# ZhaozhiQIAN/Hybrid-ODE-NeurIPS-2021

Measured on AMD Instinct MI355X. Metric: patient-trajectories/sec (fwd+adjoint) at dim=12, T=100, higher is better.
Workload: dtype f32; 1 GPU; dim12 synthetic, 10000 patients/GPU, T=100, dt=0.125, rk4(3/8), fused rhs+step kernel + discrete-adjoint kernel (split expert/learned wave pipelines); patients_total=10000, launch=hipGraph, lanes_per_patient=auto, theta_grad=True, parallelism=dp1, n_ranks=1, stage_tape=True

## Files before the change

hybrid-ode-neurips-2021_amd/csrc/hode_rk_split.hip:

```cpp
#include <hip/hip_runtime.h>
#include <stdlib.h>

#include "../../include/hode.h"
#include "hode_common.hpp"
#include "hode_host.hpp"
#include "hode_roche.hpp"

namespace hode {

#ifndef HODE_SPLIT_EXPERT_FIRST
#define HODE_SPLIT_EXPERT_FIRST 1
#endif
constexpr int kSplitPatients = 48;

struct SplitArgs {
  const float* __restrict__ t;
  const float* __restrict__ y0;
  const float* __restrict__ dosage;
  const float* __restrict__ dose_times;
  const float* __restrict__ theta;
  const float* __restrict__ w1;
  const float* __restrict__ b1;
  float* __restrict__ h;
  float* __restrict__ tape;
  unsigned long long* dbg;
  float* __restrict__ ltape;
  int* __restrict__ status;
  int B, T, K, perturb;
};

struct SpTimes {
  float t0, t1, dt, ts[4];
  HODE_DEV SpTimes(const float* __restrict__ t, int n, int perturb, int method) {
    t0 = t[n];
    t1 = t[n + 1];
    dt = t1 - t0;
    ts[0] = perturb ? nextafter_up(t0) : t0;
    ts[3] = perturb ? nextafter_down(t1) : t1;
    if (method == HODE_METHOD_RK4_38) {
      ts[1] = add_rn(t0, mul_rn(dt, (float)(1.0 / 3.0)));
      ts[2] = add_rn(t0, mul_rn(dt, (float)(2.0 / 3.0)));
    } else {
      ts[1] = add_rn(t0, mul_rn(0.5f, dt));
      ts[2] = ts[1];
    }
  }
};

template <int METHOD>
HODE_DEV float sp_stage_time(float t0, float t1, int perturb, int q) {
  const float dt = t1 - t0;
  const float c = METHOD == HODE_METHOD_RK4_38 ? (q == 1 ? (float)(1.0 / 3.0) : (q == 2 ? (float)(2.0 / 3.0) : 0.f))
                                               : (q == 0 ? 0.f : 0.5f);
  float tq = add_rn(t0, mul_rn(dt, c));
  tq = q == 3 ? t1 : tq;
  if (perturb) {
    if (q == 0) tq = nextafter_up(t0);
    if (q == 3) tq = nextafter_down(t1);
  }
  return tq;
}

constexpr int kSplitMaxT = 8192;
HODE_DEV void sp_stage_grid(float* __restrict__ tg, const float* __restrict__ t, int T) {
  for (int i = threadIdx.x; i < T + 3; i += blockDim.x) tg[i] = t[min(i, T - 1)];
}

template <int METHOD>
constexpr int sp_stages() { return METHOD == HODE_METHOD_EULER ? 1 : (METHOD == HODE_METHOD_MIDPOINT ? 2 : 4); }

template <int METHOD, class V>
HODE_DEV V sp_stage_state(int i, V y, float dt, V k1, V k2, V k3) {
  constexpr float c13 = (float)(1.0 / 3.0);
  if constexpr (METHOD == HODE_METHOD_MIDPOINT) return i == 0 ? y : vfma(k1, vsplat<V>(0.5f * dt), y);
  else if constexpr (METHOD == HODE_METHOD_RK4_38) {
    if (i == 0) return y;
    if (i == 1) return vfma(dt * k1, vsplat<V>(c13), y);
    if (i == 2) return vfma(vsplat<V>(dt), vfma(-k1, vsplat<V>(c13), k2), y);
    return vfma(vsplat<V>(dt), (k1 - k2) + k3, y);
  } else return y;
}
template <int METHOD, class V>
HODE_DEV V sp_advance(V y, float dt, V k1, V k2, V k3, V k4) {
  if constexpr (METHOD == HODE_METHOD_EULER) return vfma(vsplat<V>(dt), k1, y);
  else if constexpr (METHOD == HODE_METHOD_MIDPOINT) return vfma(vsplat<V>(dt), k2, y);
  else return vfma((k1 + 3.0f * (k2 + k3)) + k4, vsplat<V>(dt * 0.125f), y);
}

template <int V> struct IC { static constexpr int value = V; };

template <int MR> struct OwnSel { typedef float type; };
template <> struct OwnSel<2> { typedef f2 type; };

template <bool C, class A, class B> struct TypeSel { typedef A type; };
template <class A, class B> struct TypeSel<false, A, B> { typedef B type; };

#ifndef HODE_LTAPE_STAGES
#define HODE_LTAPE_STAGES 2
#endif
constexpr int kLearnedTapeStages = HODE_LTAPE_STAGES;
template <int METHOD> constexpr int sp_ltape_stages() { return METHOD == HODE_METHOD_RK4_38 ? kLearnedTapeStages : 0; }

template <int D>
struct MlRows {
  static constexpr int M = D - 4, MR = M / 4, DP = D / 2, MP = M / 2;
  static constexpr int NW = MR == 2 ? D : DP;
  static constexpr int NU = MR == 2 ? M : MP;
  static constexpr float kTanhScale = 2.885390081777927f;
  typedef typename OwnSel<MR>::type Own;
  typedef typename TypeSel<MR == 2, float, f2>::type Elem;
  struct Stage { Elem v[NW]; };
  struct Gath { Elem v[NU]; };
  f2 wp[NW];
  Own bias;
  HODE_DEV void load(const float* __restrict__ W, const float* __restrict__ b, int q) {
    if constexpr (MR == 2) {
#pragma unroll
      for (int i = 0; i < D; ++i) wp[i] = kTanhScale * pair2(W[(2 * q) * D + i], W[(2 * q + 1) * D + i]);
      bias = kTanhScale * pair2(b[2 * q], b[2 * q + 1]);
    } else {
#pragma unroll
      for (int ip = 0; ip < DP; ++ip) wp[ip] = kTanhScale * pair2(W[q * D + 2 * ip], W[q * D + 2 * ip + 1]);
      bias = kTanhScale * b[q];
    }
  }
  static HODE_DEV void gather(Own v, Elem* __restrict__ out) {
    if constexpr (MR == 2) {
      out[0] = quad_bcast<0>(v.x); out[1] = quad_bcast<0>(v.y);
      out[2] = quad_bcast<1>(v.x); out[3] = quad_bcast<1>(v.y);
      out[4] = quad_bcast<2>(v.x); out[5] = quad_bcast<2>(v.y);
      out[6] = quad_bcast<3>(v.x); out[7] = quad_bcast<3>(v.y);
    } else {
      out[0] = pair2(quad_bcast<0>(v), quad_bcast<1>(v));
      out[1] = pair2(quad_bcast<2>(v), quad_bcast<3>(v));
    }
  }
  static HODE_DEV Stage stage(const float4& e, Own Yo) {
    Stage Y;
    if constexpr (MR == 2) {
      Y.v[0] = e.x; Y.v[1] = e.y; Y.v[2] = e.z; Y.v[3] = e.w;
      gather(Yo, Y.v + 4);
    } else {
      Y.v[0] = pair2(e.x, e.y);
      Y.v[1] = pair2(e.z, e.w);
      gather(Yo, Y.v + 2);
    }
    return Y;
  }
  static HODE_DEV Own tanh_scaled(Own z) {
    if constexpr (MR == 2) {
      const f2 e = pair2(__builtin_amdgcn_exp2f(z.x), __builtin_amdgcn_exp2f(z.y)) + splat2(1.0f);
      return vfma(pair2(__builtin_amdgcn_rcpf(e.x), __builtin_amdgcn_rcpf(e.y)), splat2(-2.0f), splat2(1.0f));
    } else {
      return __builtin_fmaf(__builtin_amdgcn_rcpf(__builtin_amdgcn_exp2f(z) + 1.0f), -2.0f, 1.0f);
    }
  }
  HODE_DEV Own rhs(const Stage& Y) const {
    if constexpr (MR == 2) {
      f2 acc = bias, acc1 = splat2(0.f);
#pragma unroll
      for (int i = 0; i < D; i += 2) {
        acc = vfma(wp[i], Y.v[i], acc);
        acc1 = vfma(wp[i + 1], Y.v[i + 1], acc1);
      }
      return tanh_scaled(acc + acc1);
    } else {
      f2 acc = pair2(bias, 0.f);
#pragma unroll
      for (int ip = 0; ip < DP; ++ip) acc = vfma(wp[ip], Y.v[ip], acc);
      return tanh_scaled(hsum(acc));
    }
  }
  struct Part { f2 a, b; };
  HODE_DEV Part rhs_expert(const float4& e) const {
    Part p;
    if constexpr (MR == 2) {
      p.a = vfma(wp[2], e.z, vfma(wp[0], e.x, bias));
      p.b = vfma(wp[3], e.w, vfma(wp[1], e.y, splat2(0.f)));
    } else {
      p.a = vfma(wp[1], pair2(e.z, e.w), vfma(wp[0], pair2(e.x, e.y), pair2(bias, 0.f)));
      p.b = splat2(0.f);
    }
    return p;
  }
  HODE_DEV Own rhs_rest(const Part& p, const Stage& Y) const {
    if constexpr (MR == 2) {
      f2 acc = p.a, acc1 = p.b;
#pragma unroll
      for (int i = 4; i < D; i += 2) {
        acc = vfma(wp[i], Y.v[i], acc);
        acc1 = vfma(wp[i + 1], Y.v[i + 1], acc1);
      }
      return tanh_scaled(acc + acc1);
    } else {
      f2 acc = p.a;
#pragma unroll
      for (int ip = 2; ip < DP; ++ip) acc = vfma(wp[ip], Y.v[ip], acc);
      return tanh_scaled(hsum(acc));
    }
  }
  static HODE_DEV void outer_acc(f2 (&dw)[NW], Own u, const Stage& Y) {
#pragma unroll
    for (int i = 0; i < NW; ++i) dw[i] = vfma(u, Y.v[i], dw[i]);
  }
  static HODE_DEV float dw_at(const f2 (&dw)[NW], int r, int i) {
    if constexpr (MR == 2) return r == 0 ? dw[i].x : dw[i].y;
    else return (i & 1) ? dw[i / 2].y : dw[i / 2].x;
  }
  static HODE_DEV Own load_own(const float* __restrict__ src, int q) {
    if constexpr (MR == 2) {
      const float2 x = *reinterpret_cast<const float2*>(src + 4 + 2 * q);
      return pair2(x.x, x.y);
    } else return src[4 + q];
  }
  static HODE_DEV void store_own(float* __restrict__ dst, int q, Own v) {
    if constexpr (MR == 2) *reinterpret_cast<float2*>(dst + 4 + 2 * q) = make_float2(v.x, v.y);
    else dst[4 + q] = v;
  }
  template <int NL>
  static HODE_DEV void store_tape(float* __restrict__ dst, const Own* __restrict__ k) {
    if constexpr (MR == 2 && NL % 2 == 0) {
#pragma unroll
      for (int i = 0; i < NL; i += 2)
        *reinterpret_cast<float4*>(dst + 4 * (i / 2)) = make_float4(k[i].x, k[i].y, k[i + 1].x, k[i + 1].y);
    } else if constexpr (MR == 1 && NL == 4) {
      *reinterpret_cast<float4*>(dst) = make_float4(k[0], k[1], k[2], k[3]);
    } else if constexpr (MR == 1 && NL == 2) {
      *reinterpret_cast<float2*>(dst) = make_float2(k[0], k[1]);
    } else {
#pragma unroll
      for (int i = 0; i < NL; ++i) {
        if constexpr (MR == 2) *reinterpret_cast<float2*>(dst + 2 * i) = make_float2(k[i].x, k[i].y);
        else dst[i] = k[i];
      }
    }
  }
  template <int NL>
  static HODE_DEV void load_tape(const float* __restrict__ src, Own* __restrict__ k) {
    if constexpr (MR == 2 && NL % 2 == 0) {
#pragma unroll
      for (int i = 0; i < NL; i += 2) {
        const float4 v = *reinterpret_cast<const float4*>(src + 4 * (i / 2));
        k[i] = pair2(v.x, v.y); k[i + 1] = pair2(v.z, v.w);
      }
    } else if constexpr (MR == 1 && NL == 4) {
      const float4 v = *reinterpret_cast<const float4*>(src);
      k[0] = v.x; k[1] = v.y; k[2] = v.z; k[3] = v.w;
    } else if constexpr (MR == 1 && NL == 2) {
      const float2 v = *reinterpret_cast<const float2*>(src);
      k[0] = v.x; k[1] = v.y;
    } else {
#pragma unroll
      for (int i = 0; i < NL; ++i) {
        if constexpr (MR == 2) { const float2 v = *reinterpret_cast<const float2*>(src + 2 * i); k[i] = pair2(v.x, v.y); }
        else k[i] = src[i];
      }
    }
  }
};

template <int D, int METHOD, bool ABLATE, bool HILL2, bool K1, bool TAPE>
HODE_DEV void split_fwd_body(const SplitArgs& a) {
  constexpr int NS = sp_stages<METHOD>();
  typedef MlRows<D> Ml;
  typedef typename Ml::Own Own;
  constexpr int DP = Ml::DP;
  __shared__ __attribute__((aligned(16))) float ring[2][4][kSplitPatients][4];
  __shared__ __attribute__((aligned(16))) float dring[2][kSplitPatients][4];
  extern __shared__ float tg[];
  const int tid = threadIdx.x;
  const int wave = tid >> 6, lane = tid & 63;
  const int b0 = blockIdx.x * kSplitPatients;
  const RocheTheta th = load_theta(a.theta, ABLATE);
  const size_t row = (size_t)a.B * D;
  sp_stage_grid(tg, a.t, a.T);
#ifdef HODE_SPLIT_STAMPS
#define HODE_FSTAMP(k) if (a.dbg && blockIdx.x == 0 && lane == 0) a.dbg[(size_t)wave * a.T + (k)] = __builtin_amdgcn_s_memtime();
#else
#define HODE_FSTAMP(k)
#endif

  if (wave == 0) {
    const int slot = lane;
    const bool live = slot < kSplitPatients && b0 + slot < a.B;
    const int p = min(b0 + (slot < kSplitPatients ? slot : 0), a.B - 1);
    const int rslot = slot < kSplitPatients ? slot : 0;
    const unsigned lane_h = (unsigned)p * D, lane_t = (unsigned)p * 4;
    MlSlice<4, 1> none;
    float own1[1];
    f2 ya, yb;
    {
      const float4 v = *reinterpret_cast<const float4*>(a.y0 + (size_t)p * D);
      ya = pair2(v.x, v.y);
      yb = pair2(v.z, v.w);
      if (live) *reinterpret_cast<float4*>(a.h + (size_t)p * D) = v;
    }
    __syncthreads();
    auto e_iter = [&](int it, auto PAR) {
      constexpr int par = decltype(PAR)::value;
      if (it + 1 < a.T) {
        const float dt = tg[it + 1] - tg[it];
        const float4 dz = *reinterpret_cast<const float4*>(&dring[par][rslot][0]);
        const float dose[4] = {dz.x, dz.y, dz.z, dz.w};
        float* __restrict__ tape_it = TAPE ? a.tape + (size_t)it * (NS - 1) * a.B * 4 : nullptr;
        f2 ka[4], kb[4];
#pragma unroll
        for (int s = 0; s < 4; ++s) ka[s] = kb[s] = splat2(0.f);
#pragma unroll
        for (int s = 0; s < NS; ++s) {
          const f2 Ya = sp_stage_state<METHOD>(s, ya, dt, ka[0], ka[1], ka[2]);
          const f2 Yb = sp_stage_state<METHOD>(s, yb, dt, kb[0], kb[1], kb[2]);
          if (slot < kSplitPatients) *reinterpret_cast<float4*>(&ring[par][s][slot][0]) = make_float4(Ya.x, Ya.y, Yb.x, Yb.y);
          if constexpr (TAPE) {
            if (s >= 1)
              *reinterpret_cast<float4*>(tape_it + ((unsigned)(s - 1) * (unsigned)a.B * 4u + lane_t)) = make_float4(Ya.x, Ya.y, Yb.x, Yb.y);
          }
          const float Y[4] = {Ya.x, Ya.y, Yb.x, Yb.y};
          float k[4];
          roche_rhs<4, 1, ABLATE, HILL2>(th, none, dose[s], Y, k, own1);
          ka[s] = pair2(k[0], k[1]);
          kb[s] = pair2(k[2], k[3]);
        }
        ya = sp_advance<METHOD>(ya, dt, ka[0], ka[1], ka[2], ka[3]);
        yb = sp_advance<METHOD>(yb, dt, kb[0], kb[1], kb[2], kb[3]);
        *reinterpret_cast<float4*>(a.h + (size_t)(it + 1) * row + lane_h) = make_float4(ya.x, ya.y, yb.x, yb.y);
      }
      HODE_FSTAMP(it)
      __syncthreads();
    };
    for (int it = 0; it < a.T; it += 2) {
      e_iter(it, IC<0>{});
      if (it + 1 < a.T) e_iter(it + 1, IC<1>{});
    }
    if (a.status) {
      const bool bad = !(vfinite(ya) && vfinite(yb));
      if (bad && live) atomicOr(a.status, HODE_STATUS_NONFINITE);
    }
  } else {
    const int q = lane & 3;
    const int slot = (wave - 1) * 16 + (lane >> 2);
    const bool live = b0 + slot < a.B;
    const int p = min(b0 + slot, a.B - 1);
    Ml ml;
    ml.load(a.w1, a.b1, q);
    DoseSched<K1> ds;
    ds.dosage = a.dosage[p];
    ds.K = a.K;
    ds.taus = a.dose_times + (size_t)p * a.K;
    ds.tau0 = K1 ? ds.taus[0] : 0.f;
    auto dose_step = [&](int parity, float t0, float t1) {
      dring[parity][slot][q] = ds.at(sp_stage_time<METHOD>(t0, t1, a.perturb, q), th.kel).v;
    };
    if (a.T >= 2) dose_step(0, a.t[0], a.t[1]);
    if (a.T >= 3) dose_step(1, a.t[1], a.t[2]);
    Own yo = Ml::load_own(a.y0 + (size_t)p * D, q);
    if (live) Ml::store_own(a.h + (size_t)p * D, q, yo);
    constexpr int NLT = sp_ltape_stages<METHOD>();
    const size_t lt_step = (size_t)a.B * 4 * NLT * Ml::MR;
    const unsigned lt_lane = ((unsigned)p * 4 + q) * NLT * Ml::MR;
    __syncthreads();
    __syncthreads();
    auto m_iter = [&](int it, auto PAR) {
      constexpr int par = decltype(PAR)::value;
      const int n = it - 1;
      const float t_a = tg[it - 1], t_b = tg[it], t_c = tg[it + 1], t_d = tg[it + 2];
      const float dt = t_b - t_a;
      Own k[4];
      float4 e[4];
#pragma unroll
      for (int s = 0; s < NS; ++s) e[s] = *reinterpret_cast<const float4*>(&ring[par][s][slot][0]);
      __builtin_amdgcn_sched_barrier(0);
      dose_step(par, t_c, t_d);
#if HODE_SPLIT_EXPERT_FIRST
      typename Ml::Part pe[4];
#pragma unroll
      for (int s = 0; s < NS; ++s) pe[s] = ml.rhs_expert(e[s]);
#endif
#pragma unroll
      for (int s = 0; s < 4; ++s) k[s] = vsplat<Own>(0.f);
#pragma unroll
      for (int s = 0; s < NS; ++s) {
        const Own Yo = sp_stage_state<METHOD>(s, yo, dt, k[0], k[1], k[2]);
#if HODE_SPLIT_EXPERT_FIRST
        k[s] = ml.rhs_rest(pe[s], Ml::stage(e[s], Yo));
#else
        k[s] = ml.rhs(Ml::stage(e[s], Yo));
#endif
      }
      yo = sp_advance<METHOD>(yo, dt, k[0], k[1], k[2], k[3]);
      Ml::store_own(a.h + (size_t)(n + 1) * row + (size_t)p * D, q, yo);
      if constexpr (TAPE && NLT > 0) Ml::template store_tape<NLT>(a.ltape + (size_t)n * lt_step + lt_lane, k + (NS - NLT));
      HODE_FSTAMP(it)
      __syncthreads();
    };
    for (int it = 1; it < a.T; it += 2) {
      m_iter(it, IC<0>{});
      if (it + 1 < a.T) m_iter(it + 1, IC<1>{});
    }
    if (a.status) {
      if (!vfinite(yo) && live) atomicOr(a.status, HODE_STATUS_NONFINITE);
    }
  }
}

struct SplitBwdArgs {
  const float* __restrict__ t;
  const float* __restrict__ dosage;
  const float* __restrict__ dose_times;
  const float* __restrict__ theta;
  const float* __restrict__ w1;
  const float* __restrict__ b1;
  const float* __restrict__ h;
  const float* __restrict__ grad_h;
  float* __restrict__ grad_y0;
  float* __restrict__ part_ml;
  float* __restrict__ part_th;
  const float* __restrict__ tape;
  const float* __restrict__ ltape;
  int B, T, K, perturb;
  unsigned long long* dbg;
};

template <int METHOD, class V, class F>
HODE_DEV void sp_adjoint_step(V& lam, float dt, F&& vjp) {
  constexpr float c13 = (float)(1.0 / 3.0);
  if constexpr (METHOD == HODE_METHOD_EULER) {
    lam += vjp(0, dt * lam);
  } else if constexpr (METHOD == HODE_METHOD_MIDPOINT) {
    const V a1 = vjp(1, dt * lam);
    lam += a1;
    lam += vjp(0, (0.5f * dt) * a1);
  } else {
    const float w1 = dt * 0.125f, w3 = dt * 0.375f;
    const V a3 = vjp(3, w1 * lam);
    V da = dt * a3;
    V g1 = vfma(w1, lam, da);
    V g2 = vfma(w3, lam, -da);
    const V g = vfma(w3, lam, da);
    lam += a3;
    const V a2 = vjp(2, g);
    da = dt * a2;
    g2 += da;
    g1 = vfma(-c13, da, g1);
    lam += a2;
    const V a1 = vjp(1, g2);
    g1 = vfma(c13, dt * a1, g1);
    lam += a1;
    lam += vjp(0, g1);
  }
}

struct F4 {
  f2 a, b;
  HODE_DEV F4& operator+=(const F4& o) { a += o.a; b += o.b; return *this; }
  HODE_DEV F4 operator-() const { return F4{-a, -b}; }
};
HODE_DEV F4 operator*(float s, const F4& v) { return F4{s * v.a, s * v.b}; }
HODE_DEV F4 vfma(float s, const F4& x, const F4& y) { return F4{vfma(s, x.a, y.a), vfma(s, x.b, y.b)}; }

template <int D, bool CW>
struct SplitBwdShared {
  static constexpr int RD = CW ? 3 : 2;
  static constexpr int M = D - 4;
  float yring[RD][4][kSplitPatients][4];
  float cring[RD][4][kSplitPatients + 1][4];
  float dring[RD][kSplitPatients][8];
  float gring[RD][4][kSplitPatients + 1][4];
  float tdring[RD][kSplitPatients][8];
  float uring[CW ? RD : 1][4][CW ? kSplitPatients : 1][CW ? M : 1];
  float red[4][4][M * D + M];
};

template <int D, int METHOD, bool ABLATE, bool HILL2, bool NEED_TH, bool K1, bool TAPE>
HODE_DEV void split_bwd_body(const SplitBwdArgs& a, SplitBwdShared<D, TAPE>& sh) {
  constexpr int NS = sp_stages<METHOD>();
  typedef MlRows<D> Ml;
  typedef typename Ml::Own Own;
  constexpr int M = Ml::M, MR = Ml::MR, DP = Ml::DP, MP = Ml::MP;
  constexpr bool THW = TAPE && NEED_TH;
  constexpr bool CW = TAPE;
  constexpr int RD = SplitBwdShared<D, TAPE>::RD;
  constexpr int EL = CW ? 2 : 1;
  constexpr int CWAVE = THW ? 5 : 4;
  auto& yring = sh.yring; auto& cring = sh.cring; auto& dring = sh.dring; auto& gring = sh.gring;
  auto& tdring = sh.tdring; auto& uring = sh.uring; auto& red = sh.red;
  extern __shared__ float tg[];
  const int tid = threadIdx.x;
  const int wave = tid >> 6, lane = tid & 63;
  const int b0 = blockIdx.x * kSplitPatients;
  const RocheTheta th = load_theta(a.theta, ABLATE);
  const size_t row = (size_t)a.B * D;
  const int T = a.T;
  const int NIT = T + EL - 1;
  sp_stage_grid(tg, a.t, a.T);
#ifdef HODE_SPLIT_STAMPS
#define HODE_SSTAMP(k) if (a.dbg && blockIdx.x == 0 && lane == 0) a.dbg[(size_t)wave * (a.T + 2) + (k)] = __builtin_amdgcn_s_memtime();
#define HODE_PSTAMP(k, ph) { __builtin_amdgcn_sched_barrier(0); if (a.dbg && blockIdx.x == 0 && wave == 3 && lane == 0) a.dbg[(size_t)6 * (a.T + 2) + 64 + (size_t)(k) * 8 + (ph)] = __builtin_amdgcn_s_memtime(); __builtin_amdgcn_sched_barrier(0); }
  if (a.dbg && blockIdx.x < 8 && lane == 0) a.dbg[(size_t)6 * (a.T + 2) + blockIdx.x * 8 + wave] = __builtin_amdgcn_s_getreg(63492);
#else
#define HODE_SSTAMP(k)
#define HODE_PSTAMP(k, ph)
#endif
  auto run = [&](auto&& iter) {
    for (int k = 0; k < NIT; k += RD) {
      iter(k, IC<0>{});
      if (k + 1 < NIT) iter(k + 1, IC<1>{});
      if constexpr (RD == 3) {
        if (k + 2 < NIT) iter(k + 2, IC<2>{});
      }
    }
  };

  if (wave == 0) {
    const int slot = lane < kSplitPatients ? lane : 0;
    const bool mine = lane < kSplitPatients;
    const bool live = mine && b0 + slot < a.B;
    const int p = min(b0 + slot, a.B - 1);
    const float lv = live ? 1.0f : 0.0f;
    DoseSched<K1> ds;
    ds.dosage = a.dosage[p];
    ds.K = a.K;
    ds.taus = a.dose_times + (size_t)p * a.K;
    ds.tau0 = K1 ? ds.taus[0] : 0.f;
    const float ln_ec50 = log_f32(th.ec50);
    const int cslot = mine ? lane : kSplitPatients;
    if (lane < 16 * RD) (&cring[lane >> 4][(lane >> 2) & 3][kSplitPatients][0])[lane & 3] = 0.f;
    const unsigned lane_h = (unsigned)p * D, lane_t = (unsigned)p * 4;
    MlSlice<4, 1> none;
    MlColSlice<4, 1> nonec;
    GradAcc<4, 1> acc;
    acc.zero();
    float own1[1] = {0.f};

    float tp[4][4];
    auto fetch = [&](int m) {
      const float4 v = *reinterpret_cast<const float4*>(a.h + (size_t)m * row + lane_h);
      tp[0][0] = v.x; tp[0][1] = v.y; tp[0][2] = v.z; tp[0][3] = v.w;
      if constexpr (TAPE) {
        const float* __restrict__ tape_m = a.tape + (size_t)m * (NS - 1) * a.B * 4;
#pragma unroll
        for (int s = 1; s < NS; ++s) {
          const float4 u = *reinterpret_cast<const float4*>(tape_m + ((unsigned)(s - 1) * (unsigned)a.B * 4u + lane_t));
          tp[s][0] = u.x; tp[s][1] = u.y; tp[s][2] = u.z; tp[s][3] = u.w;
        }
      }
    };
    auto publish = [&](int m, int par) {
      if constexpr (TAPE) {
        if (mine) {
#pragma unroll
          for (int s = 0; s < NS; ++s)
            *reinterpret_cast<float4*>(&yring[par][s][slot][0]) = make_float4(tp[s][0], tp[s][1], tp[s][2], tp[s][3]);
        }
      } else {
        const SpTimes st(a.t, m, a.perturb, METHOD);
        const f2 ya = pair2(tp[0][0], tp[0][1]), yb = pair2(tp[0][2], tp[0][3]);
        f2 ka[4], kb[4];
#pragma unroll
        for (int s = 0; s < 4; ++s) ka[s] = kb[s] = splat2(0.f);
#pragma unroll
        for (int s = 0; s < NS; ++s) {
          const f2 Ya = sp_stage_state<METHOD>(s, ya, st.dt, ka[0], ka[1], ka[2]);
          const f2 Yb = sp_stage_state<METHOD>(s, yb, st.dt, kb[0], kb[1], kb[2]);
          const DoseVal dv = ds.at(st.ts[s], th.kel);
          if (mine) {
            *reinterpret_cast<float4*>(&yring[par][s][slot][0]) = make_float4(Ya.x, Ya.y, Yb.x, Yb.y);
            dring[par][slot][s] = dv.v;
            dring[par][slot][4 + s] = dv.dk;
          }
          if (s + 1 < NS) {
            const float Y[4] = {Ya.x, Ya.y, Yb.x, Yb.y};
            float k[4];
            roche_rhs<4, 1, ABLATE, HILL2>(th, none, dv.v, Y, k, own1);
            ka[s] = pair2(k[0], k[1]);
            kb[s] = pair2(k[2], k[3]);
          }
        }
      }
    };

    F4 lam;
    {
      const float4 g4 = *reinterpret_cast<const float4*>(a.grad_h + (size_t)(T - 1) * row + (size_t)p * D);
      lam.a = lv * pair2(g4.x, g4.y);
      lam.b = lv * pair2(g4.z, g4.w);
    }
    if (T >= 2) {
      fetch(T - 2);
      publish(T - 2, 0);
    }
    __syncthreads();
    auto e_iter = [&](int k, auto SI) {
      constexpr int S = decltype(SI)::value;
      constexpr int par = (S + 1) % RD;
      if (T - 3 - k >= 0) fetch(T - 3 - k);
      if (k >= EL && k <= T + EL - 2) {
        const int m = T - k + EL - 2;
        const float dt = tg[m + 1] - tg[m];
        float Y[4][4];
        F4 cs[4];
        DoseVal dv[4];
        {
          const float4 d0 = *reinterpret_cast<const float4*>(&dring[par][slot][0]);
          const float4 d1 = *reinterpret_cast<const float4*>(&dring[par][slot][4]);
          dv[0].v = d0.x; dv[1].v = d0.y; dv[2].v = d0.z; dv[3].v = d0.w;
          dv[0].dk = d1.x; dv[1].dk = d1.y; dv[2].dk = d1.z; dv[3].dk = d1.w;
          if constexpr (THW) {
            *reinterpret_cast<float4*>(&tdring[S][slot][0]) = d0;
            *reinterpret_cast<float4*>(&tdring[S][slot][4]) = d1;
          }
        }
#pragma unroll
        for (int s = 0; s < NS; ++s) {
          const float4 yv = *reinterpret_cast<const float4*>(&yring[par][s][slot][0]);
          const float4 cv = *reinterpret_cast<const float4*>(&cring[par][s][cslot][0]);
          Y[s][0] = yv.x; Y[s][1] = yv.y; Y[s][2] = yv.z; Y[s][3] = yv.w;
          cs[s].a = pair2(cv.x, cv.y);
          cs[s].b = pair2(cv.z, cv.w);
        }
        sp_adjoint_step<METHOD>(lam, dt, [&](int s, const F4& gs) {
          const float g[4] = {gs.a.x, gs.a.y, gs.b.x, gs.b.y};
          float av[4];
          if constexpr (THW) {
            if (mine) *reinterpret_cast<float4*>(&gring[S][s][slot][0]) = make_float4(g[0], g[1], g[2], g[3]);
          }
          roche_vjp<4, 1, ABLATE, HILL2, NEED_TH && !THW>(th, none, nonec, ln_ec50, dv[s], Y[s], own1, g, 0, av, acc);
          F4 r = cs[s];
          r.a += pair2(av[0], av[1]);
          r.b += pair2(av[2], av[3]);
          return r;
        });
        const float4 g4 = *reinterpret_cast<const float4*>(a.grad_h + (size_t)m * row + lane_h);
        lam.a = vfma(lv, pair2(g4.x, g4.y), lam.a);
        lam.b = vfma(lv, pair2(g4.z, g4.w), lam.b);
      }
      if (T - 3 - k >= 0) publish(T - 3 - k, par);
      HODE_SSTAMP(k)
      __syncthreads();
    };
    run(e_iter);
    if (live) *reinterpret_cast<float4*>(a.grad_y0 + (size_t)p * D) = make_float4(lam.a.x, lam.a.y, lam.b.x, lam.b.y);
    if constexpr (!THW) {
#pragma unroll
      for (int i = 0; i < kNTheta; ++i) {
        const float v = row_sum(NEED_TH ? acc.dth[i] : 0.f);
        if ((lane & 15) == 0) red[0][lane >> 4][i] = v;
      }
      __builtin_amdgcn_fence(__ATOMIC_SEQ_CST, "wavefront");
      if (lane < kNTheta)
        a.part_th[(size_t)blockIdx.x * kNTheta + lane] = (red[0][0][lane] + red[0][1][lane]) + (red[0][2][lane] + red[0][3][lane]);
    }
  } else if (THW && wave == 4) {
    const int slot = lane < kSplitPatients ? lane : 0;
    const bool mine = lane < kSplitPatients;
    const int p = min(b0 + slot, a.B - 1);
    const int gslot = mine ? lane : kSplitPatients;
    const float ln_ec50 = log_f32(th.ec50);
    if (lane < 16 * RD) (&gring[lane >> 4][(lane >> 2) & 3][kSplitPatients][0])[lane & 3] = 0.f;
    const unsigned lane_h = (unsigned)p * D, lane_t = (unsigned)p * 4;
    float dth[kNTheta];
#pragma unroll
    for (int i = 0; i < kNTheta; ++i) dth[i] = 0.f;
    float tp[4][4];
    auto fetch = [&](int m) {
      const float4 v = *reinterpret_cast<const float4*>(a.h + (size_t)m * row + lane_h);
      tp[0][0] = v.x; tp[0][1] = v.y; tp[0][2] = v.z; tp[0][3] = v.w;
      const float* __restrict__ tape_m = a.tape + (size_t)m * (NS - 1) * a.B * 4;
#pragma unroll
      for (int s = 1; s < NS; ++s) {
        const float4 u = *reinterpret_cast<const float4*>(tape_m + ((unsigned)(s - 1) * (unsigned)a.B * 4u + lane_t));
        tp[s][0] = u.x; tp[s][1] = u.y; tp[s][2] = u.z; tp[s][3] = u.w;
      }
    };
    auto theta_step = [&](int gpar) {
      const float4 d0 = *reinterpret_cast<const float4*>(&tdring[gpar][slot][0]);
      const float4 d1 = *reinterpret_cast<const float4*>(&tdring[gpar][slot][4]);
      const float dvv[4] = {d0.x, d0.y, d0.z, d0.w}, dvk[4] = {d1.x, d1.y, d1.z, d1.w};
#pragma unroll
      for (int si = 0; si < NS; ++si) {
        const int s = NS - 1 - si;
        const float4 gv = *reinterpret_cast<const float4*>(&gring[gpar][s][gslot][0]);
        DoseVal dv;
        dv.v = dvv[s]; dv.dk = dvk[s];
        const float g[4] = {gv.x, gv.y, gv.z, gv.w};
        roche_theta_grad<ABLATE, HILL2>(th, ln_ec50, dv, tp[s], g, dth);
      }
    };
    __syncthreads();
    auto t_iter = [&](int k, auto SI) {
      constexpr int S = decltype(SI)::value;
      constexpr int gpar = (S + RD - 1) % RD;
      if (k >= EL + 1) theta_step(gpar);
      if (k >= EL && T - k + EL - 2 >= 0) fetch(T - k + EL - 2);
      HODE_SSTAMP(k)
      __syncthreads();
    };
    run(t_iter);
    if (T >= 2) theta_step((NIT - 1) % RD);
#pragma unroll
    for (int i = 0; i < kNTheta; ++i) {
      const float v = row_sum(dth[i]);
      if ((lane & 15) == 0) red[0][lane >> 4][i] = v;
    }
    __builtin_amdgcn_fence(__ATOMIC_SEQ_CST, "wavefront");
    if (lane < kNTheta)
      a.part_th[(size_t)blockIdx.x * kNTheta + lane] = (red[0][0][lane] + red[0][1][lane]) + (red[0][2][lane] + red[0][3][lane]);
  } else if (CW && wave == CWAVE) {
    const int slot = lane < kSplitPatients ? lane : 0;
    const bool mine = lane < kSplitPatients;
    float wq[M][4];
#pragma unroll
    for (int j = 0; j < M; ++j)
#pragma unroll
      for (int q = 0; q < 4; ++q) wq[j][q] = a.w1[j * D + q];
    __syncthreads();
    auto c_iter = [&](int k, auto SI) {
      constexpr int S = decltype(SI)::value;
      constexpr int cpar = (S + RD - 1) % RD;
      if (k >= 1 && k - 1 <= T - 2) {
        float u[NS][M];
#pragma unroll
        for (int s = 0; s < NS; ++s) {
#pragma unroll
          for (int j4 = 0; j4 < M; j4 += 4) {
            const float4 v = *reinterpret_cast<const float4*>(&uring[cpar][s][slot][j4]);
            u[s][j4] = v.x; u[s][j4 + 1] = v.y; u[s][j4 + 2] = v.z; u[s][j4 + 3] = v.w;
          }
        }
        __builtin_amdgcn_sched_barrier(0);
#pragma unroll
        for (int s = 0; s < NS; ++s) {
          float c[4];
#pragma unroll
          for (int q = 0; q < 4; ++q) {
            if constexpr (MR == 2) {
              float cq = 0.f;
#pragma unroll
              for (int j = 0; j < M; ++j) cq = __builtin_fmaf(wq[j][q], u[s][j], cq);
              c[q] = cq;
            } else {
              float cx = 0.f, cy = 0.f;
#pragma unroll
              for (int jp = 0; jp < MP; ++jp) {
                cx = __builtin_fmaf(wq[2 * jp][q], u[s][2 * jp], cx);
                cy = __builtin_fmaf(wq[2 * jp + 1][q], u[s][2 * jp + 1], cy);
              }
              c[q] = cx + cy;
            }
          }
          if (mine) *reinterpret_cast<float4*>(&cring[cpar][s][slot][0]) = make_float4(c[0], c[1], c[2], c[3]);
        }
      }
      HODE_SSTAMP(k)
      __syncthreads();
    };
    run(c_iter);
  } else {
    const int q = lane & 3;
    const int slot = (wave - 1) * 16 + (lane >> 2);
    const bool live = b0 + slot < a.B;
    const int p = min(b0 + slot, a.B - 1);
    const float lv = live ? 1.0f : 0.0f;
    Ml ml;
    ml.load(a.w1, a.b1, q);
    typename Ml::Elem wc[Ml::NU];
    f2 wtp[Ml::NU];
    if constexpr (MR == 2) {
#pragma unroll
      for (int j = 0; j < M; ++j) {
        wc[j] = a.w1[j * D + q];
        wtp[j] = pair2(a.w1[j * D + 4 + 2 * q], a.w1[j * D + 4 + 2 * q + 1]);
      }
    } else {
#pragma unroll
      for (int jp = 0; jp < MP; ++jp) {
        wc[jp] = pair2(a.w1[(2 * jp) * D + q], a.w1[(2 * jp + 1) * D + q]);
        wtp[jp] = pair2(a.w1[(2 * jp) * D + 4 + q], a.w1[(2 * jp + 1) * D + 4 + q]);
      }
    }
    f2 dw[Ml::NW];
    Own db = vsplat<Own>(0.f);
#pragma unroll
    for (int i = 0; i < Ml::NW; ++i) dw[i] = splat2(0.f);
    DoseSched<K1> ds;
    ds.dosage = a.dosage[p];
    ds.K = a.K;
    ds.taus = a.dose_times + (size_t)p * a.K;
    ds.tau0 = K1 ? ds.taus[0] : 0.f;
    Own lam = lv * Ml::load_own(a.grad_h + (size_t)(T - 1) * row + (size_t)p * D, q);
    Own yo_nx, gh_nx;
    constexpr int NLT = TAPE ? sp_ltape_stages<METHOD>() : 0;
    const size_t lt_step = (size_t)a.B * 4 * NLT * MR;
    const unsigned lt_lane = ((unsigned)p * 4 + q) * NLT * MR;
    Own lt_nx[NLT > 0 ? NLT : 1], lt_n2[NLT > 0 ? NLT : 1];
    {
      const int m0 = T >= 2 ? T - 2 : 0;
      const int m1 = m0 >= 1 ? m0 - 1 : 0;
      yo_nx = Ml::load_own(a.h + (size_t)m0 * row + (size_t)p * D, q);
      gh_nx = Ml::load_own(a.grad_h + (size_t)m0 * row + (size_t)p * D, q);
      if constexpr (NLT > 0) {
        Ml::template load_tape<NLT>(a.ltape + (size_t)m0 * lt_step + lt_lane, lt_nx);
        Ml::template load_tape<NLT>(a.ltape + (size_t)m1 * lt_step + lt_lane, lt_n2);
      }
    }
    __syncthreads();
    auto m_iter = [&](int k, auto SI) {
      constexpr int par = decltype(SI)::value;
      if (k <= T - 2) {
        HODE_PSTAMP(k, 0)
        const int m = T - 2 - k;
        const float t0 = tg[m], t1 = tg[m + 1];
        const float dt = t1 - t0;
        const Own yo = yo_nx, gh = gh_nx;
        Own lt[NLT > 0 ? NLT : 1];
#pragma unroll
        for (int i = 0; i < NLT; ++i) { lt[i] = lt_nx[i]; lt_nx[i] = lt_n2[i]; }
        {
          const int mn = m >= 1 ? m - 1 : 0;
          yo_nx = Ml::load_own(a.h + (size_t)mn * row + (size_t)p * D, q);
          gh_nx = Ml::load_own(a.grad_h + (size_t)mn * row + (size_t)p * D, q);
          if constexpr (NLT > 0) Ml::template load_tape<NLT>(a.ltape + (size_t)(m >= 2 ? m - 2 : 0) * lt_step + lt_lane, lt_n2);
        }
        typename Ml::Stage Y[4];
        Own so[4];
        float4 e[4];
#pragma unroll
        for (int s = 0; s < NS; ++s) e[s] = *reinterpret_cast<const float4*>(&yring[par][s][slot][0]);
        __builtin_amdgcn_sched_barrier(0);
        HODE_PSTAMP(k, 1)
        if constexpr (TAPE) {
          const DoseVal dq = ds.at(sp_stage_time<METHOD>(t0, t1, a.perturb, q), th.kel);
          dring[par][slot][q] = dq.v;
          if constexpr (NEED_TH) dring[par][slot][4 + q] = dq.dk;
        }
#if HODE_SPLIT_EXPERT_FIRST
        typename Ml::Part pe[4];
#pragma unroll
        for (int s = 0; s < NS - NLT; ++s) pe[s] = ml.rhs_expert(e[s]);
#endif
#pragma unroll
        for (int s = 0; s < 4; ++s) so[s] = vsplat<Own>(0.f);
#pragma unroll
        for (int s = 0; s < NS; ++s) {
          const Own Yo = sp_stage_state<METHOD>(s, yo, dt, so[0], so[1], so[2]);
          Y[s] = Ml::stage(e[s], Yo);
          if (s >= NS - NLT) so[s] = lt[s - (NS - NLT) < 0 ? 0 : s - (NS - NLT)];
#if HODE_SPLIT_EXPERT_FIRST
          else so[s] = ml.rhs_rest(pe[s], Y[s]);
#else
          else so[s] = ml.rhs(Y[s]);
#endif
        }
        HODE_PSTAMP(k, 2)
        sp_adjoint_step<METHOD>(lam, dt, [&](int s, Own gs) {
          HODE_PSTAMP(k, 6 - s)
          const Own u = gs * vfma(-so[s], so[s], vsplat<Own>(1.0f));
          db += u;
          Ml::outer_acc(dw, u, Y[s]);
          if constexpr (CW) {
            if constexpr (MR == 2) *reinterpret_cast<float2*>(&uring[par][s][slot][2 * q]) = make_float2(u.x, u.y);
            else uring[par][s][slot][q] = u;
          }
          typename Ml::Gath uf;
          Ml::gather(u, uf.v);
          if constexpr (MR == 2) {
            float cq = 0.f;
            f2 av = splat2(0.f), av1 = splat2(0.f);
#pragma unroll
            for (int j = 0; j < M; j += 2) {
              if constexpr (!CW) cq = __builtin_fmaf(wc[j], uf.v[j], cq);
              av = vfma(wtp[j], uf.v[j], av);
              if constexpr (!CW) cq = __builtin_fmaf(wc[j + 1], uf.v[j + 1], cq);
              av1 = vfma(wtp[j + 1], uf.v[j + 1], av1);
            }
            if constexpr (!CW) cring[par][s][slot][q] = cq;
            return av + av1;
          } else {
            f2 c2 = splat2(0.f), a2 = splat2(0.f);
#pragma unroll
            for (int jp = 0; jp < MP; ++jp) {
              if constexpr (!CW) c2 = vfma(wc[jp], uf.v[jp], c2);
              a2 = vfma(wtp[jp], uf.v[jp], a2);
            }
            if constexpr (!CW) cring[par][s][slot][q] = hsum(c2);
            return hsum(a2);
          }
        });
        lam = vfma(lv, gh, lam);
        HODE_PSTAMP(k, 7)
      }
      HODE_SSTAMP(k)
      __syncthreads();
    };
    run(m_iter);
    if (live) Ml::store_own(a.grad_y0 + (size_t)p * D, q, lam);
    float* out = a.part_ml + ((size_t)blockIdx.x * 3 + (wave - 1)) * (M * D + M);
    const bool writer = (lane & 15) < 4;
    float* mine = &red[wave][lane >> 4][0];
#pragma unroll
    for (int r = 0; r < MR; ++r) {
#pragma unroll
      for (int i = 0; i < D; ++i) {
        const float v = row_sum_stride4(Ml::dw_at(dw, r, i));
        if (writer) mine[(q * MR + r) * D + i] = v;
      }
      float dbr;
      if constexpr (MR == 2) dbr = r == 0 ? db.x : db.y;
      else dbr = db;
      const float vb = row_sum_stride4(dbr);
      if (writer) mine[M * D + q * MR + r] = vb;
    }
    __builtin_amdgcn_fence(__ATOMIC_SEQ_CST, "wavefront");
    for (int c = lane; c < M * D + M; c += 64)
      out[c] = (red[wave][0][c] + red[wave][1][c]) + (red[wave][2][c] + red[wave][3][c]);
  }
}

__global__ __launch_bounds__(64) void split_fold_kernel(const float* __restrict__ part_ml, const float* __restrict__ part_th,
                                                        int nblk, int P_ml, int n_w, float* __restrict__ gw,
                                                        float* __restrict__ gb, float* __restrict__ gth, int need_th,
                                                        int overwrite) {
  const int j = blockIdx.x;
  const int lane = threadIdx.x;
  const bool ml = j < P_ml;
  const float* src = ml ? part_ml + j : part_th + (j - P_ml);
  const int rows = ml ? 3 * nblk : nblk;
  const int stride = ml ? P_ml : kNTheta;
  float s = 0.f;
  for (int base = 0; base < rows; base += 64 * 8) {
    float v[8];
#pragma unroll
    for (int q = 0; q < 8; ++q) {
      const int w = base + lane + 64 * q;
      v[q] = w < rows ? src[(size_t)w * stride] : 0.f;
    }
#pragma unroll
    for (int q = 0; q < 8; ++q) s += v[q];
  }
  s = wave_sum(s);
  if (lane != 0) return;
  float* dst = nullptr;
  if (ml) dst = j < n_w ? (gw ? gw + j : nullptr) : (gb ? gb + (j - n_w) : nullptr);
  else if (gth) dst = gth + (j - P_ml);
  if (!dst) return;
  if (!ml && !need_th) s = 0.f;
  *dst = overwrite ? s : *dst + s;
}

#ifndef HODE_SPLIT_WPE_FWD
#define HODE_SPLIT_WPE_FWD 2
#endif
#ifndef HODE_SPLIT_WPE_BWD
#define HODE_SPLIT_WPE_BWD 2
#endif
#ifndef HODE_SPLIT_WPE_BWD_MIN
#define HODE_SPLIT_WPE_BWD_MIN 1
#endif

template <int D, int METHOD, bool ABLATE, bool NEED_TH, bool TAPE>
__global__ __launch_bounds__(384) __attribute__((amdgpu_waves_per_eu(HODE_SPLIT_WPE_BWD_MIN, HODE_SPLIT_WPE_BWD))) void split_bwd_kernel(SplitBwdArgs a) {
  __shared__ __attribute__((aligned(16))) SplitBwdShared<D, TAPE> sh;
  const bool hill2 = ABLATE || (a.theta[0] == 2.0f && a.theta[1] == 2.0f);
  if (hill2 && a.K == 1) split_bwd_body<D, METHOD, ABLATE, true, NEED_TH, true, TAPE>(a, sh);
  else if (hill2) split_bwd_body<D, METHOD, ABLATE, true, NEED_TH, false, TAPE>(a, sh);
  else split_bwd_body<D, METHOD, ABLATE, false, NEED_TH, false, TAPE>(a, sh);
}

template <int D, int METHOD, bool ABLATE, bool TAPE>
__global__ __launch_bounds__(256) __attribute__((amdgpu_waves_per_eu(1, HODE_SPLIT_WPE_FWD))) void split_fwd_kernel(SplitArgs a) {
  const bool hill2 = ABLATE || (a.theta[0] == 2.0f && a.theta[1] == 2.0f);
  if (hill2 && a.K == 1) split_fwd_body<D, METHOD, ABLATE, true, true, TAPE>(a);
  else if (hill2) split_fwd_body<D, METHOD, ABLATE, true, false, TAPE>(a);
  else split_fwd_body<D, METHOD, ABLATE, false, false, TAPE>(a);
}

}

namespace {

template <int D, bool ABLATE>
int split_method(const hode_solve_desc* d, const hode::SplitArgs& a, hipStream_t s) {
  const dim3 grid((d->batch + hode::kSplitPatients - 1) / hode::kSplitPatients), block(256);
  const size_t lds = (size_t)(d->n_times + 3) * sizeof(float);
#define HODE_SPLIT_FWD(M)                                                                                 \
  if (a.tape) hipLaunchKernelGGL((hode::split_fwd_kernel<D, M, ABLATE, true>), grid, block, lds, s, a);   \
  else hipLaunchKernelGGL((hode::split_fwd_kernel<D, M, ABLATE, false>), grid, block, lds, s, a);
  switch (d->method) {
    case HODE_METHOD_EULER: HODE_SPLIT_FWD(HODE_METHOD_EULER) break;
    case HODE_METHOD_MIDPOINT: HODE_SPLIT_FWD(HODE_METHOD_MIDPOINT) break;
    default: HODE_SPLIT_FWD(HODE_METHOD_RK4_38) break;
  }
  return hode::hip_fail(hipGetLastError(), "split kernel launch");
}

}

namespace {

template <int D, bool ABLATE>
int split_bwd_method(const hode_solve_desc* d, const hode::SplitBwdArgs& a, hipStream_t s) {
  const dim3 grid((d->batch + hode::kSplitPatients - 1) / hode::kSplitPatients), block(256);
  const size_t lds = (size_t)(d->n_times + 3) * sizeof(float);
#define HODE_SPLIT_BWD(M)                                                                                        \
  if (d->need_theta_grad) {                                                                                      \
    if (a.tape) hipLaunchKernelGGL((hode::split_bwd_kernel<D, M, ABLATE, true, true>), grid, dim3(384), lds, s, a); \
    else hipLaunchKernelGGL((hode::split_bwd_kernel<D, M, ABLATE, true, false>), grid, block, lds, s, a);          \
  } else {                                                                                                       \
    if (a.tape) hipLaunchKernelGGL((hode::split_bwd_kernel<D, M, ABLATE, false, true>), grid, dim3(320), lds, s, a); \
    else hipLaunchKernelGGL((hode::split_bwd_kernel<D, M, ABLATE, false, false>), grid, block, lds, s, a);         \
  }
  switch (d->method) {
    case HODE_METHOD_EULER: HODE_SPLIT_BWD(HODE_METHOD_EULER) break;
    case HODE_METHOD_MIDPOINT: HODE_SPLIT_BWD(HODE_METHOD_MIDPOINT) break;
    default: HODE_SPLIT_BWD(HODE_METHOD_RK4_38) break;
  }
  return hode::hip_fail(hipGetLastError(), "split bwd kernel launch");
}

}

namespace hode {

bool split_supported(const hode_solve_desc* d) { return (d->latent_dim == 8 || d->latent_dim == 12) && d->n_times <= kSplitMaxT; }

static size_t al256s(size_t x) { return (x + 255) / 256 * 256; }

static int n_stages(int method) { return method == HODE_METHOD_EULER ? 1 : (method == HODE_METHOD_MIDPOINT ? 2 : 4); }

static size_t split_partials_bytes(const hode_solve_desc* d) {
  const size_t nblk = (d->batch + kSplitPatients - 1) / kSplitPatients;
  const size_t M = d->latent_dim - 4;
  return al256s(nblk * 3 * (M * d->latent_dim + M) * sizeof(float)) + al256s(nblk * kNTheta * sizeof(float));
}
static size_t split_etape_bytes(const hode_solve_desc* d) {
  if (!(d->flags & HODE_FLAG_TAPE) || d->n_times < 2) return 0;
  return al256s((size_t)(d->n_times - 1) * (n_stages(d->method) - 1) * d->batch * 4 * sizeof(float));
}
static size_t split_ltape_bytes(const hode_solve_desc* d) {
  if (!(d->flags & HODE_FLAG_TAPE) || d->n_times < 2 || n_stages(d->method) != 4 || kLearnedTapeStages == 0) return 0;
  return al256s((size_t)(d->n_times - 1) * d->batch * (d->latent_dim - 4) * kLearnedTapeStages * sizeof(float));
}
static size_t split_tape_bytes(const hode_solve_desc* d) { return split_etape_bytes(d) + split_ltape_bytes(d); }
size_t split_workspace_bytes(const hode_solve_desc* d) { return split_partials_bytes(d) + split_tape_bytes(d); }
static float* split_tape(const hode_solve_desc* d) {
  return split_etape_bytes(d) ? (float*)((char*)d->workspace + split_partials_bytes(d)) : nullptr;
}
static float* split_ltape(const hode_solve_desc* d) {
  return split_ltape_bytes(d) ? (float*)((char*)d->workspace + split_partials_bytes(d) + split_etape_bytes(d)) : nullptr;
}

int split_rk_bwd(const hode_solve_desc* d, hipStream_t s) {
  const int nblk = (d->batch + kSplitPatients - 1) / kSplitPatients;
  const int M = d->latent_dim - 4;
  const int Pml = M * d->latent_dim + M;
  char* ws = (char*)d->workspace;
  SplitBwdArgs a{};
  a.t = d->t; a.dosage = d->dosage; a.dose_times = d->dose_times; a.theta = d->theta; a.w1 = d->w1; a.b1 = d->b1;
  a.h = d->h; a.grad_h = d->grad_h; a.grad_y0 = d->grad_y0;
  a.part_ml = (float*)ws;
  a.part_th = (float*)(ws + al256s((size_t)nblk * 3 * Pml * sizeof(float)));
  a.B = d->batch; a.T = d->n_times; a.K = d->n_dose; a.perturb = d->perturb;
  a.tape = split_tape(d);
  a.ltape = split_ltape(d);
#ifdef HODE_SPLIT_STAMPS
  if (const char* env = getenv("HODE_SPLIT_DBG_PTR")) a.dbg = (unsigned long long*)strtoull(env, nullptr, 0);
#endif
  const bool abl = d->rhs_kind == HODE_RHS_ROCHE_ABLATE;
  int e;
  if (d->latent_dim == 8) e = abl ? split_bwd_method<8, true>(d, a, s) : split_bwd_method<8, false>(d, a, s);
  else e = abl ? split_bwd_method<12, true>(d, a, s) : split_bwd_method<12, false>(d, a, s);
  if (e || (d->flags & HODE_FLAG_SKIP_FOLD)) return e;
  const bool th_out = d->grad_theta != nullptr && (d->need_theta_grad || (d->flags & HODE_FLAG_OVERWRITE_GRADS));
  hipLaunchKernelGGL(split_fold_kernel, dim3(Pml + (th_out ? kNTheta : 0)), dim3(64), 0, s, a.part_ml, a.part_th, nblk, Pml,
                     M * d->latent_dim, d->grad_w1, d->grad_b1, d->grad_theta, d->need_theta_grad,
                     (d->flags & HODE_FLAG_OVERWRITE_GRADS) ? 1 : 0);
  return hip_fail(hipGetLastError(), "split_fold launch");
}

int split_rk_fwd(const hode_solve_desc* d, hipStream_t s) {
  SplitArgs a{};
  a.t = d->t; a.y0 = d->y0; a.dosage = d->dosage; a.dose_times = d->dose_times; a.theta = d->theta; a.w1 = d->w1; a.b1 = d->b1;
  a.h = d->h; a.status = d->status;
  a.B = d->batch; a.T = d->n_times; a.K = d->n_dose; a.perturb = d->perturb;
  a.tape = split_tape(d);
  a.ltape = split_ltape(d);
#ifdef HODE_SPLIT_STAMPS
  if (const char* env = getenv("HODE_SPLIT_FWD_DBG_PTR")) a.dbg = (unsigned long long*)strtoull(env, nullptr, 0);
#endif
  const bool abl = d->rhs_kind == HODE_RHS_ROCHE_ABLATE;
  if (d->latent_dim == 8) return abl ? split_method<8, true>(d, a, s) : split_method<8, false>(d, a, s);
  return abl ? split_method<12, true>(d, a, s) : split_method<12, false>(d, a, s);
}

}
```

Baseline: 76.07 million trajectories/s.

## Fuse gradient fold into adjoint kernel via last-block ticket reduction

Removes the separate split_fold kernel launch when tape and overwrite-grads are set. Each backward block stores its partials, and the last block in each of eight classes, chosen by an atomic ticket, folds that class's partials into a scratch row. The last class then writes the final weight, bias and theta gradients. Tickets are zeroed in the forward kernel. The standalone fold kernel is also reworked into an eight-way strided sum that pre-combines the three per-block ml partials. This adds atomic serialization and tail work on the final blocks and changes the floating-point summation order.

After: 74.89 million trajectories/s. 0.985x the previous value.

```diff
diff --git a/hybrid-ode-neurips-2021_amd/csrc/hode_rk_split.hip b/hybrid-ode-neurips-2021_amd/csrc/hode_rk_split.hip
--- a/hybrid-ode-neurips-2021_amd/csrc/hode_rk_split.hip
+++ b/hybrid-ode-neurips-2021_amd/csrc/hode_rk_split.hip
@@ -26,8 +26,14 @@
   unsigned long long* dbg;
   float* __restrict__ ltape;
   int* __restrict__ status;
+  unsigned* tickets;
   int B, T, K, perturb;
 };
+
+constexpr int kFoldClasses = 8;
+constexpr int kFoldTickets = 1 + kFoldClasses;
+HODE_DEV void fold_store(float* p, float v) { __hip_atomic_store(p, v, __ATOMIC_RELAXED, __HIP_MEMORY_SCOPE_AGENT); }
+HODE_DEV float fold_load(const float* p) { return __hip_atomic_load(p, __ATOMIC_RELAXED, __HIP_MEMORY_SCOPE_AGENT); }
 
 struct SpTimes {
   float t0, t1, dt, ts[4];
@@ -274,6 +280,9 @@
   const RocheTheta th = load_theta(a.theta, ABLATE);
   const size_t row = (size_t)a.B * D;
   sp_stage_grid(tg, a.t, a.T);
+  if constexpr (TAPE) {
+    if (blockIdx.x == 0 && tid < kFoldTickets) __hip_atomic_store(a.tickets + tid, 0u, __ATOMIC_RELAXED, __HIP_MEMORY_SCOPE_AGENT);
+  }
 #ifdef HODE_SPLIT_STAMPS
 #define HODE_FSTAMP(k) if (a.dbg && blockIdx.x == 0 && lane == 0) a.dbg[(size_t)wave * a.T + (k)] = __builtin_amdgcn_s_memtime();
 #else
@@ -418,6 +427,12 @@
   const float* __restrict__ tape;
   const float* __restrict__ ltape;
   int B, T, K, perturb;
+  int fuse;
+  unsigned* tickets;
+  float* cls_rows;
+  float* gw;
+  float* gb;
+  float* gth;
   unsigned long long* dbg;
 };
 
@@ -470,6 +485,63 @@
   float uring[CW ? RD : 1][4][CW ? kSplitPatients : 1][CW ? M : 1];
   float red[4][4][M * D + M];
 };
+
+template <int D, bool NEED_TH>
+HODE_DEV void split_fused_fold(const SplitBwdArgs& a, float (&red)[4][4][(D - 4) * D + (D - 4)]) {
+  constexpr int M = D - 4, Pml = M * D + M, P = Pml + kNTheta;
+  const int tid = threadIdx.x;
+  const int blk = blockIdx.x, nblk = gridDim.x;
+  const int cls = blk % kFoldClasses, ncls = min(nblk, kFoldClasses);
+  const bool ml = tid < Pml;
+  __syncthreads();
+  if (ml) fold_store(a.part_ml + (size_t)blk * 3 * Pml + tid, (red[1][0][tid] + red[2][0][tid]) + red[3][0][tid]);
+  else if (tid < P) fold_store(a.part_th + (size_t)blk * kNTheta + (tid - Pml), red[0][0][tid - Pml]);
+  __builtin_amdgcn_s_waitcnt(0);
+  __syncthreads();
+  if (tid == 0)
+    red[0][1][0] = __uint_as_float(__hip_atomic_fetch_add(a.tickets + 1 + cls, 1u, __ATOMIC_RELAXED, __HIP_MEMORY_SCOPE_AGENT));
+  __syncthreads();
+  if (__float_as_uint(red[0][1][0]) != (unsigned)((nblk - cls + kFoldClasses - 1) / kFoldClasses - 1)) return;
+  if (tid == 0) __hip_atomic_store(a.tickets + 1 + cls, 0u, __ATOMIC_RELAXED, __HIP_MEMORY_SCOPE_AGENT);
+  if (tid < P) {
+    const float* src = ml ? a.part_ml + tid : a.part_th + (tid - Pml);
+    const size_t stride = ml ? 3 * Pml : kNTheta;
+    float s = 0.f;
+    for (int b = cls; b < nblk; b += kFoldClasses * 8) {
+      float v[8];
+#pragma unroll
+      for (int q = 0; q < 8; ++q) {
+        const int bb = b + kFoldClasses * q;
+        v[q] = bb < nblk ? fold_load(src + (size_t)bb * stride) : 0.f;
+      }
+#pragma unroll
+      for (int q = 0; q < 8; ++q) s += v[q];
+    }
+    fold_store(a.cls_rows + cls * P + tid, s);
+  }
+  __builtin_amdgcn_s_waitcnt(0);
+  __syncthreads();
+  if (tid == 0)
+    red[0][2][0] = __uint_as_float(__hip_atomic_fetch_add(a.tickets, 1u, __ATOMIC_RELAXED, __HIP_MEMORY_SCOPE_AGENT));
+  __syncthreads();
+  if (__float_as_uint(red[0][2][0]) != (unsigned)(ncls - 1)) return;
+  if (tid == 0) __hip_atomic_store(a.tickets, 0u, __ATOMIC_RELAXED, __HIP_MEMORY_SCOPE_AGENT);
+  if (tid < P) {
+    float v[kFoldClasses];
+#pragma unroll
+    for (int c = 0; c < kFoldClasses; ++c) v[c] = c < ncls ? fold_load(a.cls_rows + c * P + tid) : 0.f;
+    float g = 0.f;
+#pragma unroll
+    for (int c = 0; c < kFoldClasses; ++c) g += v[c];
+    if (tid < M * D) {
+      if (a.gw) a.gw[tid] = g;
+    } else if (ml) {
+      if (a.gb) a.gb[tid - M * D] = g;
+    } else if (a.gth) {
+      a.gth[tid - Pml] = NEED_TH ? g : 0.f;
+    }
+  }
+}
 
 template <int D, int METHOD, bool ABLATE, bool HILL2, bool NEED_TH, bool K1, bool TAPE>
 HODE_DEV void split_bwd_body(const SplitBwdArgs& a, SplitBwdShared<D, TAPE>& sh) {
@@ -647,8 +719,11 @@
         if ((lane & 15) == 0) red[0][lane >> 4][i] = v;
       }
       __builtin_amdgcn_fence(__ATOMIC_SEQ_CST, "wavefront");
-      if (lane < kNTheta)
-        a.part_th[(size_t)blockIdx.x * kNTheta + lane] = (red[0][0][lane] + red[0][1][lane]) + (red[0][2][lane] + red[0][3][lane]);
+      if (lane < kNTheta) {
+        const float v = (red[0][0][lane] + red[0][1][lane]) + (red[0][2][lane] + red[0][3][lane]);
+        if (a.fuse) red[0][0][lane] = v;
+        else a.part_th[(size_t)blockIdx.x * kNTheta + lane] = v;
+      }
     }
   } else if (THW && wave == 4) {
     const int slot = lane < kSplitPatients ? lane : 0;
@@ -703,8 +778,11 @@
       if ((lane & 15) == 0) red[0][lane >> 4][i] = v;
     }
     __builtin_amdgcn_fence(__ATOMIC_SEQ_CST, "wavefront");
-    if (lane < kNTheta)
-      a.part_th[(size_t)blockIdx.x * kNTheta + lane] = (red[0][0][lane] + red[0][1][lane]) + (red[0][2][lane] + red[0][3][lane]);
+    if (lane < kNTheta) {
+      const float v = (red[0][0][lane] + red[0][1][lane]) + (red[0][2][lane] + red[0][3][lane]);
+      if (a.fuse) red[0][0][lane] = v;
+      else a.part_th[(size_t)blockIdx.x * kNTheta + lane] = v;
+    }
   } else if (CW && wave == CWAVE) {
     const int slot = lane < kSplitPatients ? lane : 0;
     const bool mine = lane < kSplitPatients;
@@ -911,8 +989,14 @@
       if (writer) mine[M * D + q * MR + r] = vb;
     }
     __builtin_amdgcn_fence(__ATOMIC_SEQ_CST, "wavefront");
-    for (int c = lane; c < M * D + M; c += 64)
-      out[c] = (red[wave][0][c] + red[wave][1][c]) + (red[wave][2][c] + red[wave][3][c]);
+    for (int c = lane; c < M * D + M; c += 64) {
+      const float v = (red[wave][0][c] + red[wave][1][c]) + (red[wave][2][c] + red[wave][3][c]);
+      if (a.fuse) red[wave][0][c] = v;
+      else out[c] = v;
+    }
+  }
+  if constexpr (TAPE) {
+    if (a.fuse) split_fused_fold<D, NEED_TH>(a, red);
   }
 }
 
@@ -924,20 +1008,26 @@
   const int lane = threadIdx.x;
   const bool ml = j < P_ml;
   const float* src = ml ? part_ml + j : part_th + (j - P_ml);
-  const int rows = ml ? 3 * nblk : nblk;
-  const int stride = ml ? P_ml : kNTheta;
+  const size_t stride = ml ? P_ml : kNTheta;
   float s = 0.f;
-  for (int base = 0; base < rows; base += 64 * 8) {
-    float v[8];
-#pragma unroll
-    for (int q = 0; q < 8; ++q) {
-      const int w = base + lane + 64 * q;
-      v[q] = w < rows ? src[(size_t)w * stride] : 0.f;
-    }
-#pragma unroll
-    for (int q = 0; q < 8; ++q) s += v[q];
-  }
-  s = wave_sum(s);
+  if (lane < kFoldClasses) {
+    for (int b = lane; b < nblk; b += kFoldClasses * 8) {
+      float v[8];
+#pragma unroll
+      for (int q = 0; q < 8; ++q) {
+        const int bb = b + kFoldClasses * q;
+        if (bb >= nblk) v[q] = 0.f;
+        else if (ml) v[q] = (src[(size_t)(3 * bb) * stride] + src[(size_t)(3 * bb + 1) * stride]) + src[(size_t)(3 * bb + 2) * stride];
+        else v[q] = src[(size_t)bb * stride];
+      }
+#pragma unroll
+      for (int q = 0; q < 8; ++q) s += v[q];
+    }
+  }
+  float g = 0.f;
+#pragma unroll
+  for (int c = 0; c < kFoldClasses; ++c) g += __shfl(s, c);
+  s = g;
   if (lane != 0) return;
   float* dst = nullptr;
   if (ml) dst = j < n_w ? (gw ? gw + j : nullptr) : (gb ? gb + (j - n_w) : nullptr);
@@ -1027,10 +1117,18 @@
 
 static int n_stages(int method) { return method == HODE_METHOD_EULER ? 1 : (method == HODE_METHOD_MIDPOINT ? 2 : 4); }
 
+static size_t split_fold_scratch_bytes(const hode_solve_desc* d) {
+  const size_t M = d->latent_dim - 4;
+  return 256 + al256s(kFoldClasses * (M * d->latent_dim + M + kNTheta) * sizeof(float));
+}
 static size_t split_partials_bytes(const hode_solve_desc* d) {
   const size_t nblk = (d->batch + kSplitPatients - 1) / kSplitPatients;
   const size_t M = d->latent_dim - 4;
-  return al256s(nblk * 3 * (M * d->latent_dim + M) * sizeof(float)) + al256s(nblk * kNTheta * sizeof(float));
+  return al256s(nblk * 3 * (M * d->latent_dim + M) * sizeof(float)) + al256s(nblk * kNTheta * sizeof(float)) +
+         split_fold_scratch_bytes(d);
+}
+static char* split_fold_scratch(const hode_solve_desc* d) {
+  return (char*)d->workspace + split_partials_bytes(d) - split_fold_scratch_bytes(d);
 }
 static size_t split_etape_bytes(const hode_solve_desc* d) {
   if (!(d->flags & HODE_FLAG_TAPE) || d->n_times < 2) return 0;
@@ -1062,6 +1160,10 @@
   a.B = d->batch; a.T = d->n_times; a.K = d->n_dose; a.perturb = d->perturb;
   a.tape = split_tape(d);
   a.ltape = split_ltape(d);
+  a.fuse = a.tape != nullptr && (d->flags & HODE_FLAG_OVERWRITE_GRADS) && !(d->flags & HODE_FLAG_SKIP_FOLD);
+  a.tickets = a.fuse ? (unsigned*)split_fold_scratch(d) : nullptr;
+  a.cls_rows = a.fuse ? (float*)(split_fold_scratch(d) + 256) : nullptr;
+  a.gw = d->grad_w1; a.gb = d->grad_b1; a.gth = d->grad_theta;
 #ifdef HODE_SPLIT_STAMPS
   if (const char* env = getenv("HODE_SPLIT_DBG_PTR")) a.dbg = (unsigned long long*)strtoull(env, nullptr, 0);
 #endif
@@ -1069,7 +1171,7 @@
   int e;
   if (d->latent_dim == 8) e = abl ? split_bwd_method<8, true>(d, a, s) : split_bwd_method<8, false>(d, a, s);
   else e = abl ? split_bwd_method<12, true>(d, a, s) : split_bwd_method<12, false>(d, a, s);
-  if (e || (d->flags & HODE_FLAG_SKIP_FOLD)) return e;
+  if (e || (d->flags & HODE_FLAG_SKIP_FOLD) || a.fuse) return e;
   const bool th_out = d->grad_theta != nullptr && (d->need_theta_grad || (d->flags & HODE_FLAG_OVERWRITE_GRADS));
   hipLaunchKernelGGL(split_fold_kernel, dim3(Pml + (th_out ? kNTheta : 0)), dim3(64), 0, s, a.part_ml, a.part_th, nblk, Pml,
                      M * d->latent_dim, d->grad_w1, d->grad_b1, d->grad_theta, d->need_theta_grad,
@@ -1084,6 +1186,7 @@
   a.B = d->batch; a.T = d->n_times; a.K = d->n_dose; a.perturb = d->perturb;
   a.tape = split_tape(d);
   a.ltape = split_ltape(d);
+  a.tickets = a.tape ? (unsigned*)split_fold_scratch(d) : nullptr;
 #ifdef HODE_SPLIT_STAMPS
   if (const char* env = getenv("HODE_SPLIT_FWD_DBG_PTR")) a.dbg = (unsigned long long*)strtoull(env, nullptr, 0);
 #endif
```
